# phlash/java-sdr

Hardware: AMD Instinct MI355X
Metric: IQ Msamples/s through FFT+FIR+BPSK demod, 2048-pt frames (higher is better)
Workload: dtype f64

## Files before the change

### java-sdr_amd/build.py

```python
#!/usr/bin/env python3
import os
import subprocess
import sys
from concurrent.futures import ThreadPoolExecutor

HERE = os.path.dirname(os.path.abspath(__file__))
CSRC = os.path.join(HERE, "csrc")
OBJ = os.path.join(HERE, "build")
OUT = os.path.join(HERE, "libjsdr_hip.so")

COMMON = ["--offload-arch=gfx950", "-O3", "-std=c++17", "-fPIC", "-Wall", "-Wno-unused-function",
          "-Wno-unused-result"]
SOURCES = {
    "bpsk_front_reg.hip": ["-ffp-contract=off"],
    "bpsk_fm.hip": ["-ffp-contract=off"],
    "bpsk_fm_f32.hip": ["-ffp-contract=off"],
    "bpsk_front.hip": ["-ffp-contract=off"],
    "bpsk_tail.hip": ["-ffp-contract=off"],
    "runtime.hip": [],
    "fft_psd.hip": [],
    "fft_mixed.hip": [],
    "fft_any.hip": ["-ffp-contract=off"],
    "fft_rt.hip": [],
    "fir_phase.hip": ["-ffp-contract=off"],
    "fir_batch.hip": ["-ffp-contract=off"],
    "fec.hip": [],
    "synth.hip": [],
    "formats.hip": [],
    "demod.hip": ["-ffp-contract=off"],
    "demod_chan.hip": ["-ffp-contract=off"],
    "bpsk_handle.hip": ["-ffp-contract=off"],
    "bpsk_sched.hip": ["-ffp-contract=off"],
    "bpsk_fft.hip": ["-ffp-contract=off"],
    "bpsk_acq.hip": ["-ffp-contract=off", "-mllvm", "-amdgpu-atomic-optimizer-strategy=None"],
    "bpsk_acq_chan.hip": ["-ffp-contract=off", "-mllvm", "-amdgpu-atomic-optimizer-strategy=None"],
    "bpsk_fftm.hip": ["-ffp-contract=off"],
    "bpsk_acqg.hip": ["-ffp-contract=off"],
    "bpsk_chan.hip": ["-ffp-contract=off"],
    "bpsk_pst.hip": ["-ffp-contract=off"],
# ... 57 lines not shown
```

### java-sdr_amd/csrc/bpsk_fm.hip

```cpp
#include "bpsk_units.h"
#include "bpsk_tuner.h"
#include <math.h>
#include <type_traits>
#include <stddef.h>
#include <stdlib.h>

namespace jsdr {
namespace fm { __constant__ BpskConst c_bpsk; }
using fm::c_bpsk;
}
#include "bpsk_matched.h"

namespace jsdr {


template <bool FAST>
__global__ __launch_bounds__(512) void k_matched(MatchedArgs a)
{
    extern __shared__ __align__(16) unsigned char smem[];
    double2 *X = reinterpret_cast<double2 *>(smem);
    const int s = blockIdx.y;
    const long long G = a.tile0 + 4160LL * blockIdx.x;
    const double2 *dm = a.dm + (long long)s * a.dm_stride;
    {
// ... 42 lines not shown
__global__ __launch_bounds__(64) void k_dm_history(double2 *dm, long long dm_stride, long long nds, int nstreams)
{
    int s = blockIdx.x;
    if (s >= nstreams) return;
    double2 *p = dm + (long long)s * dm_stride;
    double2 v = p[nds + threadIdx.x];
    __builtin_amdgcn_fence(__ATOMIC_RELEASE, "wavefront");
    __builtin_amdgcn_wave_barrier();
    asm volatile("s_waitcnt vmcnt(0)" ::: "memory");
    p[threadIdx.x] = v;
}


#ifdef JSDR_X_CLK
__device__ unsigned long long g_fm_clk[256][64];
#define FM_CLK(i)                                                                          \
    do {                                                                                   \
        const unsigned long long now_ = __builtin_amdgcn_s_memtime();                      \
        clk_acc_[i] += now_ - clk_last_;                                                   \
        clk_last_ = now_;                                                                  \
    } while (0)
#else
#define FM_CLK(i) do {} while (0)
#endif

__global__ void k_fm_edges(EdgeArgs a)
{
    const int t = blockIdx.x * blockDim.x + threadIdx.x;
    const int s = t / (4 * FM_EDGE), i = t % (4 * FM_EDGE);
    if (s >= a.nstreams) return;
    const int n = i < 2 * FM_EDGE ? i - FM_EDGE : a.nsamples - FM_EDGE + (i - 2 * FM_EDGE);
    int w = 0;
    if (n >= 0 && n < a.nsamples) {
        w = a.raw[(long long)s * a.stride_pairs + n];
    } else if (n < 0 && n >= -26) {
        w = a.hist[(long long)s * 32 + 26 + n].x;
        if (a.dc) {
            const int si = (int)(short)((w & 0xffff) - a.ic);
            const int sq = (int)(short)((w >> 16) - a.qc);
            w = (si & 0xffff) | (sq << 16);
        }
    }
    a.edges[(long long)s * (4 * FM_EDGE) + i] = w;
}

__global__ void k_fm_prep(EdgeArgs e, HistArgs hi, ScatterArgs sc)
// ... 48 lines not shown
        if (k != (float)(int)k || k >= 16384.0f || k <= -16384.0f) return false;
    }
    return true;
}
static_assert(ds_taps_are_short(), "dsFilter: every tap times 2^15 is an integer of magnitude below 2^14 (k_fm's +-1.0 fmas are exact)");

template <int D, int R, bool MIX, bool DC, bool FAST, bool SMALL = false, int PH = -1>
#ifndef JSDR_FM_MINWAVES
#define JSDR_FM_MINWAVES 2
#endif
__global__ __launch_bounds__(FM_THREADS, JSDR_FM_MINWAVES) void k_fm(FmArgs a)
{
    constexpr int RD = D * R, NS = RD - D + 27, NSQ = (NS + 3) / 4;
    constexpr int JOBS = (FM_NT + R - 1) / R, ROUNDS = (JOBS + FM_THREADS - 1) / FM_THREADS;
    static_assert(PH < 0 || (MIX && !FAST && PH < 4 && (D * R) % 8 == 0 && (65 * FM_NB * D) % 8 == 4),
                  "k_fm<PH>: the lane span is whole periods and a tile is half a period past the one before");
    extern __shared__ __align__(16) unsigned char smem[];
    double2 *X = reinterpret_cast<double2 *>(smem);
    double *sc = reinterpret_cast<double *>(smem + FM_NT * sizeof(double2));
    for (int i = threadIdx.x; i < 512; i += FM_THREADS) sc[i] = a.sincos[i];
#ifdef JSDR_X_CLK
    unsigned long long clk_acc_[6] = {0, 0, 0, 0, 0, 0}, clk_last_ = 0;
#endif
    const long long nwork = (long long)a.ntiles * a.nstreams;
#pragma unroll 1
    for (long long work = blockIdx.x; work < nwork; work += gridDim.x) {
    const int s = (int)(work / a.ntiles);
    const long long G = a.tile0 + (long long)(65 * FM_NB) * (work % a.ntiles);
    const int jrel0 = (int)(G - 64 - a.g_first);
#ifdef JSDR_X_FM_SMALLSET
    const int *raw = a.raw + (long long)(s & 15) * a.stride_pairs;
#else
    const int *raw = a.raw + (long long)s * a.stride_pairs;
#endif
    const int *edges = a.edges + (long long)s * (4 * FM_EDGE);
    const double2 *dmh_old = a.dmh_old + (long long)s * 64;
    const int Lm1 = a.nsamples - 1, nds = a.nds, P = a.tper;
    const double HOWARD = 0.9 * 32768.0 * (double)I16_2P15_UNSCALE;
    int e0 = 0;
    if constexpr (MIX) {
        const long long v = (long long)a.first_out + (long long)D * jrel0;
        e0 = (int)(((v % P) + P) % P);
    }
    typedef const __attribute__((address_space(4))) double *const_tab_t;
    const_tab_t tb = (const_tab_t)(a.tcs + e0);
    float amx = 0.0f;
    __syncthreads();
#ifdef JSDR_X_CLK
    clk_last_ = __builtin_amdgcn_s_memtime();
// ... 122 lines not shown
#pragma unroll 1
            for (int r = 0; r < R; r++) {
                const int t = t0 + r, j = j0 + r;
                const double2 val = (j >= -64 && j < 0) ? dmh_old[64 + j] : make_double2(0.0, 0.0);
                if (t < FM_NT) X[t] = val;
            }
        }
    }
    };
    if constexpr (PH < 0) {
        front(std::integral_constant<int, -1>{});
    } else {
        if (((e0 + a.trot) & 7) == PH) front(std::integral_constant<int, PH>{});
        else front(std::integral_constant<int, PH + 4>{});
    }
    if constexpr (FAST) {
#pragma unroll
        for (int off = 32; off >= 1; off >>= 1) amx = fmaxf(amx, __shfl_xor(amx, off, 64));
        if ((threadIdx.x & 63) == 0 && amx > 0.0f) atomicMax(a.amax + s, __float_as_int(amx));
    }
    FM_CLK(1);
    __syncthreads();
    FM_CLK(3);
    if (jrel0 + FM_NT > nds - 64) {
        double2 *dmh_new = a.dmh_new + (long long)s * 64;
        for (int t = 64 + threadIdx.x; t < FM_NT; t += FM_THREADS) {
            const int j = jrel0 + t;
            if (j >= nds - 64 && j < nds && j >= 0) dmh_new[j - (nds - 64)] = X[t];
        }
        if (work % a.ntiles == 0 && nds < 64 && (int)threadIdx.x < 64 - nds) dmh_new[threadIdx.x] = dmh_old[threadIdx.x + nds];
    }
    const int lane = threadIdx.x & 63;
    const int wave = __builtin_amdgcn_readfirstlane(threadIdx.x >> 6);
    const int blk = lane < FM_NB ? lane : FM_NB - 1;
    const double2 *xl = X + 64 + 65 * blk;
    const int rel0 = jrel0 + 64 + 65 * blk;
    double2 *y = a.y + (long long)s * a.y_stride;
    if constexpr (SMALL) {
        const int rel = (int)threadIdx.x, t = rel - jrel0;
        if (rel < nds && t >= 64 && t < FM_NT) {
            const long long g = a.g_first + rel;
            const int u = (int)(((g - 64) % 65 + 65) % 65);
            const double2 *xg = X + t;
            const double *f = c_bpsk.dm_taps;
            double yi = 0.0, yq = 0.0;
            for (int i = 0; i <= 64 - u; i++) {
// ... 56 lines not shown
    }
#else
    if (wave == 0) {
        double ai[9], aq[9];
        matched_block<9, FAST>(xl, 0, ai, aq);
#pragma unroll
        for (int r = 0; r < 9; r++) {
            const int rel = rel0 + r;
            if (lane < FM_NB && rel >= 0 && rel < nds) y[rel] = make_double2(ai[r], aq[r]);
        }
    } else {
        const int u0 = 9 + 8 * (wave - 1);
        double ai[8], aq[8];
        matched_block<8, FAST>(xl, u0, ai, aq);
#pragma unroll
        for (int r = 0; r < 8; r++) {
            const int rel = rel0 + u0 + r;
            if (lane < FM_NB && rel >= 0 && rel < nds) y[rel] = make_double2(ai[r], aq[r]);
        }
    }
#endif
    }
    FM_CLK(4);
    __syncthreads();
    FM_CLK(5);
    }
#ifdef JSDR_X_CLK
    if ((threadIdx.x & 63) == 0)
        for (int i = 0; i < 6; i++) atomicAdd(&g_fm_clk[blockIdx.x & 255][(threadIdx.x >> 6) * 8 + i], clk_acc_[i]);
#endif
}


int bpsk_fm_upload_constants(const BpskConst &bc)
{
    JSDR_HIP_TRY(hipMemcpyToSymbol(HIP_SYMBOL(c_bpsk), &bc, sizeof(bc)));
    return JSDR_OK;
}

int launch_matched(const MatchedArgs &ma, int nstreams, hipStream_t st)
{
    const long long ntiles = (ma.g_first + ma.nds - ma.tile0 + 4159) / 4160;
    const size_t lds = (64 + 4160) * sizeof(double2);
    JSDR_LDS_ATTR(k_matched<false>, lds);
    JSDR_LDS_ATTR(k_matched<true>, lds);
    hipLaunchKernelGGL(k_matched<false>, dim3((unsigned)ntiles, (unsigned)nstreams), dim3(512), lds, st, ma);
    return launched();
}

int launch_dm_history(double2 *dm, long long dm_stride, long long nds, int nstreams, hipStream_t st)
{
    hipLaunchKernelGGL(k_dm_history, dim3((unsigned)nstreams), dim3(64), 0, st, dm, dm_stride, nds, nstreams);
    return launched();
}

int launch_fm_prep(const EdgeArgs &ea, const HistArgs &ha, const ScatterArgs &sc, hipStream_t st)
{
    hipLaunchKernelGGL(k_fm_prep, dim3((unsigned)(((long long)ea.nstreams * (4 * FM_EDGE + 32) + sc.bytes[0] + sc.bytes[1] + 255) / 256)),
                       dim3(256), 0, st, ea, ha, sc);
    return launched();
}

template <int D, int R>
static int launch_fm_t(const FmArgs &a_in, bool mix, bool dc, bool fast, int nstreams, hipStream_t st, long long *items, long long *grid_out,
                       int *phase)
{
    *phase = -1;
    const size_t lds = (size_t)FM_NT * sizeof(double2) + 512 * sizeof(double);
    const long long span = 65LL * FM_NB;
    const long long ntiles = (a_in.g_first + a_in.nds - a_in.tile0 + span - 1) / span;
    FmArgs a = a_in;
    a.ntiles = (int)ntiles;
    a.nstreams = nstreams;
    static const long long grid_cap = [] {
        const char *e = knob("JSDR_FM_GRID");
        return e ? atoll(e) : 0LL;
    }();
    long long gx = ntiles * nstreams;
    if (grid_cap > 0 && gx > grid_cap) gx = grid_cap;
    if (a.grid_limit > 0 && gx > a.grid_limit) gx = a.grid_limit;
    *items = ntiles * nstreams;
    *grid_out = gx;
    const dim3 grid((unsigned)gx), block(FM_THREADS);
#define JSDR_FM_LAUNCH_PH(MIX, DC, FAST, SMALL, PH)                                                             \
    do {                                                                                                        \
        JSDR_LDS_ATTR((k_fm<D, R, MIX, DC, FAST, SMALL, PH>), lds);                                             \
        hipLaunchKernelGGL((k_fm<D, R, MIX, DC, FAST, SMALL, PH>), grid, block, lds, st, a);                    \
    } while (0)
#define JSDR_FM_LAUNCH(MIX, DC, FAST, SMALL) JSDR_FM_LAUNCH_PH(MIX, DC, FAST, SMALL, -1)
    const bool small = !fast && a.nds <= FM_THREADS && ntiles == 1;
    if constexpr (D == 10) {
        if (mix && !fast && !small && a.trot >= 0 && a.tper == 8) {
            const long long v = (long long)a.first_out + (long long)D * (a.tile0 - 64 - a.g_first);
            const int p0 = (int)((((v % 8) + 8) % 8 + a.trot) & 7);
            *phase = p0;
            switch (p0 & 3) {
                case 0: if (dc) JSDR_FM_LAUNCH_PH(true, true, false, false, 0); else JSDR_FM_LAUNCH_PH(true, false, false, false, 0); break;
                case 1: if (dc) JSDR_FM_LAUNCH_PH(true, true, false, false, 1); else JSDR_FM_LAUNCH_PH(true, false, false, false, 1); break;
                case 2: if (dc) JSDR_FM_LAUNCH_PH(true, true, false, false, 2); else JSDR_FM_LAUNCH_PH(true, false, false, false, 2); break;
                default: if (dc) JSDR_FM_LAUNCH_PH(true, true, false, false, 3); else JSDR_FM_LAUNCH_PH(true, false, false, false, 3); break;
            }
            return launched();
        }
    }
    if (small && a.nds <= FM_THREADS && ntiles == 1) {
// ... 6 lines not shown
        if (mix) { if (dc) JSDR_FM_LAUNCH(true, true, false, false); else JSDR_FM_LAUNCH(true, false, false, false); }
        else { if (dc) JSDR_FM_LAUNCH(false, true, false, false); else JSDR_FM_LAUNCH(false, false, false, false); }
    }
#undef JSDR_FM_LAUNCH
#undef JSDR_FM_LAUNCH_PH
    return launched();
}

int launch_fm(const FmArgs &a, int decim, bool mix, bool dc, bool fast, int nstreams, hipStream_t st, long long *items, long long *grid,
              int *phase)
{
    switch (decim) {
        case 4: return launch_fm_t<4, 5>(a, mix, dc, fast, nstreams, st, items, grid, phase);
        case 5: return launch_fm_t<5, 4>(a, mix, dc, fast, nstreams, st, items, grid, phase);
        case 10: return launch_fm_t<10, 4>(a, mix, dc, fast, nstreams, st, items, grid, phase);
        case 20: return launch_fm_t<20, 4>(a, mix, dc, fast, nstreams, st, items, grid, phase);
    }
    set_error("bpsk: unsupported decimation %d", decim);
    return JSDR_ERR;
}

void bpsk_fm_clocks_report()
{
#ifdef JSDR_X_CLK
    {
        static unsigned long long cc[256][64];
        if (hipMemcpyFromSymbol(cc, HIP_SYMBOL(g_fm_clk), sizeof(cc)) == hipSuccess) {
            static const char *nm[6] = {"-", "front half", "-", "barrier front", "matched", "barrier matched"};
            for (int i = 0; i < 6; i++) {
                if (i == 0 || i == 2) continue;
                fprintf(stderr, "k_fm clk %-16s", nm[i]);
                for (int w = 0; w < 8; w++) {
                    unsigned long long c = 0, tot = 0;
                    for (int b = 0; b < 256; b++) {
                        c += cc[b][w * 8 + i];
                        for (int k = 0; k < 6; k++) tot += cc[b][w * 8 + k];
                    }
                    fprintf(stderr, " w%d %5.1f%%", w, 100.0 * c / (tot ? tot : 1));
                }
                fprintf(stderr, "\n");
            }
            memset(cc, 0, sizeof(cc));
            hipMemcpyToSymbol(HIP_SYMBOL(g_fm_clk), cc, sizeof(cc));
        }
    }
#endif
// ... 4 lines not shown
```

### java-sdr_amd/csrc/bpsk_fm_f32.hip

```cpp
#include "bpsk_units.h"
#include <math.h>
#include <stddef.h>
#include <stdlib.h>

namespace jsdr {
namespace fm32 { __constant__ BpskConst c_bpsk; }
using fm32::c_bpsk;
}
#include "bpsk_matched.h"

namespace jsdr {

#ifndef JSDR_FM32_PQ
#define JSDR_FM32_PQ 6
#endif
enum { FM32_PQ = JSDR_FM32_PQ };

__global__ void k_fm_prep_f32(EdgeF32Args e, HistArgs hi)
{
    const int t = blockIdx.x * blockDim.x + threadIdx.x;
    const int nedge = e.nstreams * 4 * FM_EDGE;
    if (t < nedge) {
        const int s = t / (4 * FM_EDGE), i = t % (4 * FM_EDGE);
        const int n = i < 2 * FM_EDGE ? i - FM_EDGE : e.nsamples - FM_EDGE + (i - 2 * FM_EDGE);
// ... 14 lines not shown
    int2 v;
    if (n < 0) {
        v = hi.hist_old[(long long)s * 32 + (26 + n)];
    } else {
        const float2 f = hi.rawf[(long long)s * hi.stride_pairs + n];
        v = make_int2(__float_as_int(f.x), __float_as_int(f.y));
    }
    hi.hist_new[(long long)s * 32 + i] = v;
}

template <int D, int R, bool MIX, bool SMALL = false>
__global__ __launch_bounds__(FM_THREADS, 2) void k_fm_f32(FmF32Args fa)
{
    const FmArgs &a = fa.a;
    constexpr int RD = D * R, NS = RD - D + 27, NQ = (NS + 1) / 2;
    constexpr int PQ = FM32_PQ, NP = (NQ + PQ - 1) / PQ;
    constexpr int JOBS = (FM_NT + R - 1) / R, ROUNDS = (JOBS + FM_THREADS - 1) / FM_THREADS;
    static_assert(2 * NQ <= FM_EDGE, "a window must fit an edge image's half");
    extern __shared__ __align__(16) unsigned char smem[];
    double2 *X = reinterpret_cast<double2 *>(smem);
    double *sc = reinterpret_cast<double *>(smem + FM_NT * sizeof(double2));
    for (int i = threadIdx.x; i < 512; i += FM_THREADS) sc[i] = a.sincos[i];
    const long long nwork = (long long)a.ntiles * a.nstreams;
#pragma unroll 1
    for (long long work = blockIdx.x; work < nwork; work += gridDim.x) {
    const int s = (int)(work / a.ntiles);
    const long long G = a.tile0 + (long long)(65 * FM_NB) * (work % a.ntiles);
    const int jrel0 = (int)(G - 64 - a.g_first);
    const float2 *raw = fa.rawf + (long long)s * a.stride_pairs;
    const float2 *edges = fa.edges + (long long)s * (4 * FM_EDGE);
    const double2 *dmh_old = a.dmh_old + (long long)s * 64;
    const int Lm1 = a.nsamples - 1, nds = a.nds, P = a.tper;
    const double HOWARD = 0.9 * 32768.0;
    int e0 = 0;
    if constexpr (MIX) {
        const long long v = (long long)a.first_out + (long long)D * jrel0;
        e0 = (int)(((v % P) + P) % P);
    }
    typedef const __attribute__((address_space(4))) double *const_tab_t;
    const_tab_t tb = (const_tab_t)(a.tcs + e0);
    __syncthreads();
#pragma unroll 1
    for (int round = 0; round < ROUNDS; round++) {
        const int job = threadIdx.x + FM_THREADS * round;
        const int t0 = R * job;
        if (t0 >= FM_NT) break;
        const int j0 = jrel0 + t0;
        const int n0 = a.first_out + D * j0 - 26;
// ... 100 lines not shown
#pragma unroll 1
                for (int r = 0; r < R; r++) {
                    const int t = t0 + r, j = j0 + r;
                    double2 val = make_double2(0.0, 0.0);
                    if (j >= 0 && j < nds) {
                        val.x = r == 0 ? oi[0] : r == 1 ? oi[1] : r == 2 ? oi[2] : r == 3 ? oi[3] : oi[R - 1];
                        val.y = r == 0 ? oq[0] : r == 1 ? oq[1] : r == 2 ? oq[2] : r == 3 ? oq[3] : oq[R - 1];
                    } else if (j >= -64 && j < 0) {
                        val = dmh_old[64 + j];
                    }
                    if (t < FM_NT) X[t] = val;
                }
            }
        } else {
#pragma unroll 1
            for (int r = 0; r < R; r++) {
                const int t = t0 + r, j = j0 + r;
                const double2 val = (j >= -64 && j < 0) ? dmh_old[64 + j] : make_double2(0.0, 0.0);
                if (t < FM_NT) X[t] = val;
            }
        }
    }
    __syncthreads();
    if (jrel0 + FM_NT > nds - 64) {
        double2 *dmh_new = a.dmh_new + (long long)s * 64;
        for (int t = 64 + threadIdx.x; t < FM_NT; t += FM_THREADS) {
            const int j = jrel0 + t;
            if (j >= nds - 64 && j < nds && j >= 0) dmh_new[j - (nds - 64)] = X[t];
        }
        if (work % a.ntiles == 0 && nds < 64 && (int)threadIdx.x < 64 - nds) dmh_new[threadIdx.x] = dmh_old[threadIdx.x + nds];
    }
    const int lane = threadIdx.x & 63;
    const int wave = __builtin_amdgcn_readfirstlane(threadIdx.x >> 6);
    const int blk = lane < FM_NB ? lane : FM_NB - 1;
    const double2 *xl = X + 64 + 65 * blk;
    double2 *y = a.y + (long long)s * a.y_stride;
    if constexpr (SMALL) {
        const int rel = (int)threadIdx.x, t = rel - jrel0;
        if (rel < nds && t >= 64 && t < FM_NT) {
            const long long g = a.g_first + rel;
            const int u = (int)(((g - 64) % 65 + 65) % 65);
            const double2 *xg = X + t;
            const double *f = c_bpsk.dm_taps;
            double yi = 0.0, yq = 0.0;
            for (int i = 0; i <= 64 - u; i++) {
                const double2 x = xg[-(u + i)];
// ... 18 lines not shown
            u0 = 9 + 8 * (wave - 1);
            nout = 8;
            double bi[8], bq[8];
            matched_block<8, false>(xl, u0, bi, bq);
#pragma unroll
            for (int r = 0; r < 8; r++) {
                ai[r] = bi[r];
                aq[r] = bq[r];
            }
        }
        __syncthreads();
        if (lane < FM_NB) {
#pragma unroll
            for (int r = 0; r < 9; r++)
                if (r < nout) X[65 * blk + u0 + r] = make_double2(ai[r], aq[r]);
        }
        __syncthreads();
        const int relb = jrel0 + 64;
        for (int o = (int)threadIdx.x; o < 65 * FM_NB; o += FM_THREADS) {
            const int rel = relb + o;
            if (rel >= 0 && rel < nds) y[rel] = X[o];
        }
    }
    __syncthreads();
    }
}

int bpsk_fm_f32_upload_constants(const BpskConst &bc)
{
    JSDR_HIP_TRY(hipMemcpyToSymbol(HIP_SYMBOL(c_bpsk), &bc, sizeof(bc)));
    return JSDR_OK;
}

int launch_fm_prep_f32(const EdgeF32Args &ea, const HistArgs &ha, hipStream_t st)
{
    hipLaunchKernelGGL(k_fm_prep_f32, dim3((unsigned)(((long long)ea.nstreams * (4 * FM_EDGE + 32) + 255) / 256)), dim3(256), 0, st, ea, ha);
    return launched();
}

template <int D, int R>
static int launch_fm_f32_t(const FmF32Args &a_in, bool mix, int nstreams, hipStream_t st, long long *items, long long *grid_out)
{
    const size_t lds = (size_t)FM_NT * sizeof(double2) + 512 * sizeof(double);
    const long long span = 65LL * FM_NB;
    const long long ntiles = (a_in.a.g_first + a_in.a.nds - a_in.a.tile0 + span - 1) / span;
    FmF32Args a = a_in;
    a.a.ntiles = (int)ntiles;
    a.a.nstreams = nstreams;
    long long gx = ntiles * nstreams;
    if (a.a.grid_limit > 0 && gx > a.a.grid_limit) gx = a.a.grid_limit;
    *items = ntiles * nstreams;
    *grid_out = gx;
    const dim3 grid((unsigned)gx), block(FM_THREADS);
#define JSDR_FM32_LAUNCH(MIX, SMALL)                                              \
    do {                                                                          \
        JSDR_LDS_ATTR((k_fm_f32<D, R, MIX, SMALL>), lds);                         \
        hipLaunchKernelGGL((k_fm_f32<D, R, MIX, SMALL>), grid, block, lds, st, a); \
    } while (0)
    if (a.a.nds <= FM_THREADS && ntiles == 1) {
        if (mix) JSDR_FM32_LAUNCH(true, true); else JSDR_FM32_LAUNCH(false, true);
    } else {
        if (mix) JSDR_FM32_LAUNCH(true, false); else JSDR_FM32_LAUNCH(false, false);
    }
#undef JSDR_FM32_LAUNCH
    return launched();
}

int launch_fm_f32(const FmF32Args &a, int decim, bool mix, int nstreams, hipStream_t st, long long *items, long long *grid)
{
    switch (decim) {
        case 4: return launch_fm_f32_t<4, 5>(a, mix, nstreams, st, items, grid);
        case 5: return launch_fm_f32_t<5, 4>(a, mix, nstreams, st, items, grid);
        case 10: return launch_fm_f32_t<10, 4>(a, mix, nstreams, st, items, grid);
        case 20: return launch_fm_f32_t<20, 4>(a, mix, nstreams, st, items, grid);
    }
// ... 6 lines not shown
```

### java-sdr_amd/csrc/bpsk_handle.hip

```cpp
#include "bpsk_kernels.h"
#include "bpsk_fec.h"
#include "bpsk_fft.h"
#include "bpsk_chan.h"
#include "bpsk_pst.h"
#include "bpsk_sched.h"
#include "bpsk_blob.h"
#include "bpsk_state.h"
#include <math.h>
#include <cmath>
#include <atomic>
#include <memory>
#include <thread>
#include <stddef.h>
#include <stdlib.h>
#include <vector>

static const float h_ds_half[14] = {-6.103515625000e-004F, -1.220703125000e-004F, +2.380371093750e-003F,
                                    +6.164550781250e-003F, +7.324218750000e-003F, +7.629394531250e-004F,
                                    -1.464843750000e-002F, -3.112792968750e-002F, -3.225708007813e-002F,
                                    -1.617431640625e-003F, +6.463623046875e-002F, +1.502380371094e-001F,
                                    +2.231445312500e-001F, +2.518310546875e-001F};
static const float h_dm_half[33] = {
    -0.0101130691F, -0.0086975143F, -0.0038246093F, +0.0033563764F, +0.0107237026F, +0.0157790936F, +0.0164594107F,
    +0.0119213911F, +0.0030315224F, -0.0076488191F, -0.0164594107F, -0.0197184277F, -0.0150109226F, -0.0023082460F,
// ... 36 lines not shown
    Schedule cur, prefetch;
    bool tables_on_device = false;
    unsigned char h_khist[26] = {0};
    bool retuned = false;
    bool fft_ready = false;
    int seam = 0;
    DevBuf<FftFrontState> fft_state2;
    DevBuf<double2> dm2;
    long long dm2_stride = 0;
    unsigned char h_mhist[26] = {0};
    DevBuf<unsigned short> ktu9;
    DevBuf<double> sincos9;
    std::vector<unsigned short> h_ktu9;
    int c_kshift = -1;
    DevBuf<double> sincos;
    DevBuf<unsigned char> ktu;
    DevBuf<unsigned char> kvco;
    DevBuf<int2> hist_in[2];
    int hist_cur = 0;
    bool hist_is_float = false;
    DevBuf<int> hist_bad;
    DevBuf<int> amax;
    DevBuf<SnapPack> snap_dev;
    DevBuf<int> fm_edges;
    DevBuf<float2> fm_edges_f32;
    bool f32_batch = false;
    DevBuf<double2> dm, y[2];
    int y_cur = 0;
    DevBuf<double2> dmh[2], tcs;
    int dmh_cur = 0;
    int tab_cur = 0;
    bool halo_in_dmh = false;
    bool use_fm = true;
    long long last_fm_items = 0, last_fm_grid = 0;
    int last_fm_phase = -1;
    int share_wgs_per_cu = 0;
    int num_cu = 0;
    int variant = 0;
    double fast_ey = 0.0;
    double margin_scale = 1.0;
    double argmax_scale = 1.0;
    const char *front_name = "k_front";
    const char *tail_name = "k_tail";
    const char *fec_name = "k_fec_bpsk";
    bool ktu_uploaded = false;
    std::thread worker;
// ... 1193 lines not shown
    } else if (nds > 0 && fm_ok) {
        if (wait_tail(h, h->y_cur, st) != JSDR_OK) return JSDR_ERR;
        FmArgs ma;
        ma.raw = fa.raw;
        ma.stride_pairs = fa.stride_pairs;
        ma.nsamples = (int)L;
        ma.ic = ic;
        ma.qc = qc;
        ma.edges = h->fm_edges.p;
        ma.tcs = tcs_p;
        ma.tper = h->cur.mix ? h->cur.tper : 1;
        ma.kvco = kvco_p;
        ma.sincos = h->sincos.p;
        ma.dmh_old = h->dmh[h->dmh_cur].p;
        ma.dmh_new = h->dmh[h->dmh_cur ^ 1].p;
        ma.y = h->y[h->y_cur].p + Y_PAD;
        ma.y_stride = h->y_stride;
        ma.nds = (int)nds;
        ma.g_first = g_first;
        ma.tile0 = first_block(g_first);
        ma.first_out = first_out;
        ma.amax = h->amax.p;
        ma.grid_limit = h->share_wgs_per_cu * h->num_cu;
        ma.trot = h->cur.mix == 1 ? h->cur.trot : -1;
        if (rawf_dev) {
            EdgeF32Args ea;
            ea.rawf = fa.rawf;
            ea.stride_pairs = fa.stride_pairs;
            ea.nsamples = (int)L;
            ea.hist = fa.hist;
            ea.edges = h->fm_edges_f32.p;
            ea.nstreams = S;
            const HistArgs ha = hist_args(h, nullptr, fa.rawf, fa.stride_pairs, L, 0, 0, S);
            ProfScope psh(h, PK_PREP, st);
            if (launch_fm_prep_f32(ea, ha, st) != JSDR_OK) return JSDR_ERR;
            hist_done = true;
        } else {
            EdgeArgs ea;
            ea.raw = fa.raw;
            ea.stride_pairs = fa.stride_pairs;
            ea.nsamples = (int)L;
            ea.ic = ic;
            ea.qc = qc;
            ea.dc = (ic != 0) || (qc != 0);
            ea.hist = fa.hist;
            ea.edges = h->fm_edges.p;
// ... 212 lines not shown
    if (const char *e = knob("JSDR_NO_OVERLAP")) h->overlap = atoi(e) == 0;
    if (const char *e = knob("JSDR_FM")) h->use_fm = atoi(e) != 0;
    if (const char *e = knob("JSDR_SCHED_PREFETCH")) h->prefetch_on = atoi(e) != 0;
    const size_t S = (size_t)nstreams;
    bool vitq = nstreams >= 256;
    if (const char *e = knob("JSDR_VITQ")) vitq = atoi(e) != 0 && nstreams > 1;
    h->dm_stride = 64 + h->max_ds + 64;
    h->y_stride = h->max_ds;
    h->bitlog_stride = (HIST_BITS + h->max_bits + 64 + 15) & ~15LL;
    bool ok = h->sincos.alloc(512) == JSDR_OK && h->ktu.alloc((size_t)h->max_batch + 8192) == JSDR_OK &&
              h->kvco.alloc(2 * (size_t)h->max_ds) == JSDR_OK && h->hist_in[0].alloc(S * 32) == JSDR_OK &&
              h->hist_in[1].alloc(S * 32) == JSDR_OK && h->dm.alloc(S * (size_t)h->dm_stride) == JSDR_OK &&
              h->y[0].alloc(S * (size_t)h->y_stride + 2 * Y_PAD) == JSDR_OK && h->y[1].alloc(S * (size_t)h->y_stride + 2 * Y_PAD) == JSDR_OK && h->tail.alloc(S) == JSDR_OK &&
              h->bitlog[0].alloc(S * (size_t)h->bitlog_stride) == JSDR_OK &&
              h->bitlog[1].alloc(S * (size_t)h->bitlog_stride) == JSDR_OK && h->nbits.alloc(S) == JSDR_OK &&
              h->trig_count.alloc(S) == JSDR_OK && h->trig_bits.alloc(S * h->trig_cap) == JSDR_OK &&
              h->fec_scratch.alloc(vitq ? (size_t)fec_vitq_scratch_words(nstreams, h->trig_cap) : S * h->trig_cap * (size_t)fec_dec_scratch_words()) == JSDR_OK && h->fec_done.alloc(S) == JSDR_OK &&
              (!vitq || (h->fec_vit.alloc(S * h->trig_cap * 320) == JSDR_OK && h->fec_work.alloc(S * h->trig_cap + 1) == JSDR_OK)) &&
              h->fec_rc.alloc(S * h->trig_cap) == JSDR_OK && h->fec_last.alloc(S * 2) == JSDR_OK &&
              h->cnt_dec.alloc(S) == JSDR_OK && h->corr.alloc(S * (size_t)h->max_bits) == JSDR_OK &&
              h->fec_data.alloc(S * h->trig_cap * 256) == JSDR_OK && h->decoded.alloc(S * 256) == JSDR_OK &&
              h->stage_raw.alloc((size_t)nsamples_per_frame * 2 + (nstreams == 1 ? ((do_fft ? sizeof(double2) : 1) * (size_t)h->max_ds + sizeof(double2) * (256 + FM_TABLE_SLACK) + 256) / 4 : 0)) == JSDR_OK &&
              h->ds_taps_dev.alloc(32) == JSDR_OK &&
              h->dmh[0].alloc(S * 64) == JSDR_OK && h->dmh[1].alloc(S * 64) == JSDR_OK && h->hist_bad.alloc(1) == JSDR_OK && h->amax.alloc(S) == JSDR_OK && h->fm_edges.alloc(S * 4 * FM_EDGE) == JSDR_OK && h->snap_dev.alloc(1) == JSDR_OK && h->tcs.alloc(2 * (256 + FM_TABLE_SLACK)) == JSDR_OK;
    if (ok && nstreams == 1) {
        const size_t need = sizeof(float) * 2 * (size_t)nsamples_per_frame + ((size_t)h->max_batch + 26) + (size_t)h->max_ds +
                            (do_fft ? sizeof(double2) * (size_t)h->max_ds : 0) + sizeof(double2) * (256 + FM_TABLE_SLACK) + 8 * 64;
        const size_t arena = (need + 63) & ~(size_t)63;
        if (arena <= ((size_t)8 << 20) && h->pin.alloc(arena + sizeof(SnapPack))) h->pin_bytes = arena;
        else (void)hipGetLastError();
    }
    if (!ok) {
        jsdr_bpsk_destroy(h);
        return JSDR_ERR;
    }
    std::vector<double> sc(512);
    for (int n = 0; n < 256; n++) {
        sc[n] = table_cos(n);
        sc[256 + n] = table_sin(n);
    }
    BpskConst bc;
    memset(&bc, 0, sizeof(bc));
    double sync[SYNC_N];
    (void)jsdr_bpsk_table(0, bc.ds_taps, 32);
    (void)jsdr_bpsk_table(1, bc.dm_taps, 96);
    (void)jsdr_bpsk_table(2, sync, SYNC_N);
    for (int i = 0; i < SYNC_N; i++) bc.sync[i] = sync[i] > 0.0 ? 1 : -1;
// ... 1534 lines not shown
```

### java-sdr_amd/csrc/bpsk_kernels.h

```cpp
#pragma once
#include "common.h"
#include "bpsk_fft.h"

namespace jsdr {

enum { DS_N = 27, DM_N = 65, HIST_BITS = 5200, MIN_TRIG = 8, SYNC_N = 65 };
enum { Y_PAD = 1024 };
#ifndef JSDR_FM_NB
#define JSDR_FM_NB 62
#endif
enum { FM_NB = JSDR_FM_NB, FM_NT = 64 + 65 * FM_NB, FM_THREADS = 512, FM_TABLE_SLACK = 128, FM_EDGE = 128 };

struct BpskConst {
    double ds_taps[32];
    double dm_taps[96];
    signed char sync[72];
};
int bpsk_upload_constants(const BpskConst &bc);

struct TailState {
    double dmEnergy[8];
    double dmEnergyOut;
    double lastI, lastQ;
    double energy1, energy2;
// ... 58 lines not shown
};

struct FmArgs {
    const int *raw;
    long long stride_pairs;
    int nsamples;
    int ic, qc;
    const int *edges;
    const double2 *tcs;
    int tper;
    const unsigned char *kvco;
    const double *sincos;
    const double2 *dmh_old;
    double2 *dmh_new;
    double2 *y;
    long long y_stride;
    int nds;
    long long g_first;
    long long tile0;
    int first_out;
    int *amax;
    int ntiles, nstreams;
    int grid_limit;
    int trot;
};

struct EdgeArgs {
    const int *raw;
    long long stride_pairs;
    int nsamples, ic, qc, dc;
    const int2 *hist;
    int *edges;
    int nstreams;
};
struct ScatterArgs {
    const unsigned char *src[2];
    unsigned char *dst[2];
    int bytes[2];
};

struct FmF32Args {
    FmArgs a;
    const float2 *rawf;
    const float2 *edges;
};
struct EdgeF32Args {
// ... 91 lines not shown
```

### java-sdr_amd/csrc/fft_common.h

```cpp
#pragma once
#include "common.h"
#include <utility>
#include <vector>

namespace jsdr {

constexpr double cx_pi = 3.14159265358979323846264338327950288;

constexpr double cx_sin_small(double x)
{
    double x2 = x * x, term = x, sum = x;
    for (int i = 1; i < 12; i++) {
        term *= -x2 / ((2 * i) * (2 * i + 1));
        sum += term;
    }
    return sum;
}
constexpr double cx_cos_small(double x)
{
    double x2 = x * x, term = 1.0, sum = 1.0;
    for (int i = 1; i < 12; i++) {
        term *= -x2 / ((2 * i - 1) * (2 * i));
        sum += term;
    }
// ... 78 lines not shown
    int o = 0;
    for (int b = 1; b < r; b <<= 1) {
        o = (o << 1) | (v & 1);
        v >>= 1;
    }
    return o;
}

__device__ __forceinline__ int lds_pad(int idx) { return idx + (idx >> 4); }
constexpr int lds_frame_elems(int n) { return n + (n >> 4) + 1; }


enum { IN_I16 = 0, IN_F32 = 1 };
enum { OUT_PSD = 0, OUT_SPEC = 1 };

struct FftArgs {
    const void *in;
    float *out;
    const float2 *tw;
    long long nframes;
    int rate;
    int ic, qc;
    int split = 0;
};

struct Best {
    float v;
    int k;
};

struct MixedPlan {
    int n = 0, nrad = 0, radix[6] = {1, 1, 1, 1, 1, 1};
    int threads = 0;
    size_t lds_bytes = 0;
    int tw_count = 0;
    bool split2 = false;
    int half_tw_count = 0;
};
bool mixed_plan(int n, MixedPlan &p);
void mixed_twiddles(const MixedPlan &p, float2 *out);
int mixed_launch(const MixedPlan &p, const FftArgs &a, int in_kind, int out_kind, int grid, hipStream_t st);
int mixed_launch_split2(const MixedPlan &p, const FftArgs &a, int in_kind, int out_kind, int num_cu, hipStream_t st);

bool rt_supported(int n);
void rt_twiddles(int n, std::vector<float2> &w);
int rt_launch(const FftArgs &a, int n, int in_kind, int out_kind, int num_cu, hipStream_t st);
// ... 6 lines not shown
```

### java-sdr_amd/csrc/fft_psd.hip

```cpp
#include "fft_common.h"
#include <math.h>
#include <stdlib.h>
#include <vector>

namespace jsdr {

constexpr bool tw_direct(int P, int R) { return P * R <= 512; }
constexpr int tw_size(int P, int R) { return P <= 1 ? 0 : (tw_direct(P, R) ? 2 * P * (R - 1) : P); }
constexpr int tw_total(int R0, int R1, int R2, int R3)
{
    return tw_size(R0, R1) + (R2 > 1 ? tw_size(R0 * R1, R2) : 0) + (R3 > 1 ? tw_size(R0 * R1 * R2, R3) : 0);
}

constexpr int ilog2_c(int n) { return n <= 1 ? 0 : 1 + ilog2_c(n / 2); }

template <int R, int P>
__device__ __forceinline__ void apply_twiddles(float2 *v, int k, const float2 *tab)
{
    if constexpr (P > 1) {
        if constexpr (tw_direct(P, R)) {
#pragma unroll
            for (int r = 1; r < R; r++) {
                const float4 t = reinterpret_cast<const float4 *>(tab)[(r - 1) * P + k];
                v[r] = cmul2(v[r], make_float2(t.x, t.y), make_float2(t.z, t.w));
// ... 193 lines not shown
                for (int w = 1; w < NW; w++) {
                    float ov = red_val[frame_in_block * NW + w];
                    int ok = red_idx[frame_in_block * NW + w];
                    if (ov > bestv || (ov == bestv && ok < bestk)) {
                        bestv = ov;
                        bestk = ok;
                    }
                }
            }
        }
        if (tid == 0 && active) {
            int p = (bestv > -3.402823466e+38f) ? 2 * bestk : -1;
            float m = (p >= 0) ? bestv : -3.402823466e+38f;
            const int datlen = 2 * N;
            if (p >= datlen / 2) p -= datlen;
            int hz = (int)((unsigned)p * (unsigned)a.rate) / datlen;
            float *dst = a.out + frame * (N + 2);
            dst[N] = (float)hz;
            dst[N + 1] = m;
        }
    }
}

template <int N, int T, int FPB, int IN, int OUT, int R0, int R1, int R2, int R3, bool TWG = false>
__global__ __launch_bounds__(T *FPB, (N == 2048 ? 4 : 1)) void k_fft(FftArgs a)
{
    extern __shared__ __align__(16) unsigned char smem[];
    constexpr int FE = lds_frame_elems(N);
    constexpr int TWN = TWG ? 0 : tw_total(R0, R1, R2, R3);
    float2 *tw_own = reinterpret_cast<float2 *>(smem);
    float2 *bufs = tw_own + TWN;
    float *red_val = reinterpret_cast<float *>(bufs + (size_t)FPB * FE);
    int *red_idx = reinterpret_cast<int *>(red_val + FPB * ((T + 63) / 64));
    const float2 *tw_lds = TWG ? a.tw : tw_own;

    const int tid_b = threadIdx.x;
    if constexpr (!TWG) {
        for (int i = tid_b; i < TWN; i += T * FPB) tw_own[i] = a.tw[i];
        __syncthreads();
    }

    const int fib = tid_b / T;
    const int tid = tid_b - fib * T;
    float2 *buf = bufs + (size_t)fib * FE;
    const long long ngroups = (a.nframes + FPB - 1) / FPB;
    auto frame_of = [&](long long g) {
        long long f = g * FPB + fib;
        return f < a.nframes ? f : a.nframes - 1;
    };
    typename RawPoint<IN>::type raw[R0];
    if ((long long)blockIdx.x < ngroups) fft_fetch<N, T, IN, R0>(a, frame_of(blockIdx.x), tid, raw);
    for (long long g = blockIdx.x; g < ngroups; g += gridDim.x) {
        const long long gn = g + gridDim.x;
        fft_frame<N, T, IN, OUT, R0, R1, R2, R3>(a, frame_of(g), frame_of(gn < ngroups ? gn : g), tid, buf, tw_lds, red_val,
                                                 red_idx, fib, raw);
        __syncthreads();
    }
}

template <int N, int FPB, int T, int R0, int R1, int R2, int R3, bool TWG = false>
constexpr size_t fft_lds_bytes()
{
    return sizeof(float2) * ((TWG ? (size_t)0 : (size_t)tw_total(R0, R1, R2, R3)) + (size_t)FPB * lds_frame_elems(N)) +
           (sizeof(float) + sizeof(int)) * FPB * ((T + 63) / 64);
}

struct Launcher {
    void (*launch)(const FftArgs &, int grid, hipStream_t) = nullptr;
    int frames_per_block = 0;
    size_t lds_bytes = 0;
    int block = 0;
    int radix[4] = {1, 1, 1, 1};
};

template <int N, int T, int FPB, int IN, int OUT, int R0, int R1, int R2, int R3, bool TWG = false>
static void launch_impl(const FftArgs &a, int grid, hipStream_t s)
{
    constexpr size_t lds = fft_lds_bytes<N, FPB, T, R0, R1, R2, R3, TWG>();
    hipLaunchKernelGGL((k_fft<N, T, FPB, IN, OUT, R0, R1, R2, R3, TWG>), dim3(grid), dim3(T * FPB), lds, s, a);
}
// ... 31 lines not shown
}

}

using namespace jsdr;

struct jsdr_fft {
    int n = 0;
    int rate = 0;
    DevBuf<float2> tw;
    DevBuf<float2> tw_i16;
    DevBuf<unsigned char> in_stage;
    DevBuf<float> out_stage;
    PinnedStage pin;
    bool pin_lazy_done = false;
    int num_cu = 256;
    bool mixed = false;
    MixedPlan mplan;
    bool rt = false;
    bool direct = false;
    long long last_items = 0, last_grid = 0;
    int share_wgs_per_cu = 0;
};

static int fft_run(jsdr_fft *h, const void *in_dev, int in_kind, int out_kind, long long nframes, int ic, int qc,
                   float *out_dev, hipStream_t s)
{
    JSDR_REQUIRE(h, "fft: null handle");
    JSDR_REQUIRE(in_dev && out_dev, "fft: null buffer");
    JSDR_REQUIRE(nframes >= 0, "fft: negative frame count");
    if (nframes == 0) return JSDR_OK;
    FftArgs a;
    if (h->rt) {
        a.in = in_dev;
        a.out = out_dev;
        a.tw = h->tw.p;
        a.nframes = nframes;
        a.rate = h->rate;
        a.ic = ic;
        a.qc = qc;
        return rt_launch(a, h->n, in_kind, out_kind, h->num_cu, s);
    }
    if (h->direct) {
        a.in = in_dev;
        a.out = out_dev;
        a.tw = nullptr;
// ... 25 lines not shown
    a.nframes = nframes;
    a.rate = h->rate;
    a.ic = ic;
    a.qc = qc;
    long long groups = (nframes + l.frames_per_block - 1) / l.frames_per_block;
    long long per_cu = (long long)(160 * 1024 / l.lds_bytes);
    if (per_cu < 1) per_cu = 1;
    if (per_cu * l.block > 2048) per_cu = 2048 / l.block;
    static const int mult = [] {
        const char *e = knob("JSDR_FFT_GRID_MULT");
        const int v = e ? atoi(e) : 0;
        return v > 0 ? v : 4;
    }();
    long long cap = (long long)h->num_cu * per_cu * mult;
    static const int abs_grid = [] {
        const char *e = knob("JSDR_FFT_GRID_ABS");
        return e ? atoi(e) : 0;
    }();
    if (abs_grid > 0) cap = abs_grid;
    if (h->share_wgs_per_cu > 0) cap = (long long)h->num_cu * h->share_wgs_per_cu;
    int grid = (int)(groups < cap ? groups : cap);
    h->last_items = groups;
    h->last_grid = grid;
    l.launch(a, grid, s);
    JSDR_LAUNCH_CHECK();
    return JSDR_OK;
}

extern "C" {

int jsdr_fft_create(jsdr_fft **out, int n, int rate)
{
    JSDR_REQUIRE(out, "jsdr_fft_create: null handle pointer");
    *out = nullptr;
    MixedPlan mp;
    const bool pow2 = n >= 64 && n <= 8192 && (n & (n - 1)) == 0;
    const bool mixed = !pow2 && mixed_plan(n, mp);
    const bool rt = !pow2 && !mixed && rt_supported(n);
    const bool direct = !pow2 && !mixed && !rt && dft_any_supported(n);
    JSDR_REQUIRE(pow2 || mixed || rt || direct,
                 "jsdr_fft_create: n=%d unsupported (2 .. 20000 samples)", n);
    JSDR_REQUIRE(rate > 0, "jsdr_fft_create: rate must be positive");
    int dev = 0;
    JSDR_HIP_TRY(hipGetDevice(&dev));
    hipDeviceProp_t prop;
    JSDR_HIP_TRY(hipGetDeviceProperties(&prop, dev));
// ... 67 lines not shown
        return JSDR_ERR;
    }
    std::vector<float2> tw16(tw);
    if (fft_i16_scaled(l.radix[0], l.radix[1]))
        for (int i = 0; i < tw_size(l.radix[0], l.radix[1]); i++)
            tw16[i] = make_float2(tw16[i].x * I16_2P15_UNSCALE, tw16[i].y * I16_2P15_UNSCALE);
    if (h->tw.alloc(tw.size()) != JSDR_OK || h->tw_i16.alloc(tw16.size()) != JSDR_OK ||
        h->in_stage.alloc((size_t)n * 8) != JSDR_OK || h->out_stage.alloc((size_t)n + 2) != JSDR_OK) {
        jsdr_fft_destroy(h);
        return JSDR_ERR;
    }
    if (hipMemcpy(h->tw.p, tw.data(), sizeof(float2) * tw.size(), hipMemcpyHostToDevice) != hipSuccess ||
        hipMemcpy(h->tw_i16.p, tw16.data(), sizeof(float2) * tw16.size(), hipMemcpyHostToDevice) != hipSuccess) {
        set_error("jsdr_fft_create: twiddle upload failed");
        jsdr_fft_destroy(h);
        return JSDR_ERR;
    }
    *out = h;
    return JSDR_OK;
}

int jsdr_fft_destroy(jsdr_fft *h)
{
    delete h;
    return JSDR_OK;
}

int jsdr_fft_batch_f32(jsdr_fft *h, const float *iq_dev, int64_t nframes, float *psd_dev, void *stream)
{
    return fft_run(h, iq_dev, IN_F32, OUT_PSD, nframes, 0, 0, psd_dev, as_stream(stream));
}

int jsdr_fft_set_cu_share(jsdr_fft *h, int wgs_per_cu)
{
    JSDR_REQUIRE(h && wgs_per_cu >= 0 && wgs_per_cu <= 16, "jsdr_fft_set_cu_share: bad argument");
    h->share_wgs_per_cu = wgs_per_cu;
    return JSDR_OK;
}

const char *jsdr_fft_kernel(jsdr_fft *h)
{
    if (!h) return "";
    return h->rt ? "k_fft_rt" : h->direct ? "k_dft_any" : h->mixed ? (h->mplan.split2 ? "k_fft_mixed_dual" : "k_fft_mixed") : "k_fft";
}

int jsdr_fft_last_launch(jsdr_fft *h, int64_t *work_items, int64_t *workgroups)
// ... 60 lines not shown
```

Baseline: 241,600.

## Use atomic ticket work-stealing for persistent FM kernel tiles when grid is capped

Replaces the static grid-stride tile assignment in the persistent FM kernels (f64 and f32) with dynamic tickets from a global atomic counter, broadcast through an LDS slot. This applies only when a CU-share grid limit caps the grid below the work count. The aim is to balance uneven per-tile work across workgroups and cut tail idle time, at the cost of one atomic per tile and a memset per launch. It also adds compile-gated per-workgroup clock instrumentation for FM and FFT.

```diff
diff --git a/java-sdr_amd/build.py b/java-sdr_amd/build.py
--- a/java-sdr_amd/build.py
+++ b/java-sdr_amd/build.py
@@ -13,8 +13,8 @@
           "-Wno-unused-result"]
 SOURCES = {
     "bpsk_front_reg.hip": ["-ffp-contract=off"],
-    "bpsk_fm.hip": ["-ffp-contract=off"],
-    "bpsk_fm_f32.hip": ["-ffp-contract=off"],
+    "bpsk_fm.hip": ["-ffp-contract=off", "-mllvm", "-amdgpu-atomic-optimizer-strategy=None"],
+    "bpsk_fm_f32.hip": ["-ffp-contract=off", "-mllvm", "-amdgpu-atomic-optimizer-strategy=None"],
     "bpsk_front.hip": ["-ffp-contract=off"],
     "bpsk_tail.hip": ["-ffp-contract=off"],
     "runtime.hip": [],
diff --git a/java-sdr_amd/csrc/bpsk_fm.hip b/java-sdr_amd/csrc/bpsk_fm.hip
--- a/java-sdr_amd/csrc/bpsk_fm.hip
+++ b/java-sdr_amd/csrc/bpsk_fm.hip
@@ -88,6 +88,12 @@
     } while (0)
 #else
 #define FM_CLK(i) do {} while (0)
+#endif
+
+#ifdef JSDR_X_WGCLK
+constexpr int WGCLK_SLOTS = 128, WGCLK_WGS = 1024;
+__device__ unsigned long long g_fm_wgclk[WGCLK_SLOTS][WGCLK_WGS][3];
+static long long g_wgclk_log[WGCLK_SLOTS][4];
 #endif
 
 __global__ void k_fm_edges(EdgeArgs a)
@@ -182,9 +188,15 @@
 #ifdef JSDR_X_CLK
     unsigned long long clk_acc_[6] = {0, 0, 0, 0, 0, 0}, clk_last_ = 0;
 #endif
+#ifdef JSDR_X_WGCLK
+    const unsigned long long wgclk0 = __builtin_amdgcn_s_memrealtime();
+    unsigned long long wgclk_n = 0;
+#endif
     const long long nwork = (long long)a.ntiles * a.nstreams;
+    const bool tickets = a.tickets != nullptr;
+    int *tkL = reinterpret_cast<int *>(sc + 512);
 #pragma unroll 1
-    for (long long work = blockIdx.x; work < nwork; work += gridDim.x) {
+    for (long long work = blockIdx.x; work < nwork; work = tickets ? (long long)gridDim.x + (unsigned)__builtin_amdgcn_readfirstlane(tkL[0]) : work + gridDim.x) {
     const int s = (int)(work / a.ntiles);
     const long long G = a.tile0 + (long long)(65 * FM_NB) * (work % a.ntiles);
     const int jrel0 = (int)(G - 64 - a.g_first);
@@ -353,6 +365,8 @@
     FM_CLK(1);
     __syncthreads();
     FM_CLK(3);
+    unsigned tk = 0;
+    if (tickets && threadIdx.x == 0) tk = atomicAdd(a.tickets, 1u);
     if (jrel0 + FM_NT > nds - 64) {
         double2 *dmh_new = a.dmh_new + (long long)s * 64;
         for (int t = 64 + threadIdx.x; t < FM_NT; t += FM_THREADS) {
@@ -455,9 +469,25 @@
 #endif
     }
     FM_CLK(4);
+    {
+        int zlate = 0;
+        asm volatile("" : "+v"(zlate));
+        if (tickets && threadIdx.x == 0) tkL[0] = (int)tk + zlate;
+    }
     __syncthreads();
     FM_CLK(5);
-    }
+#ifdef JSDR_X_WGCLK
+    wgclk_n++;
+#endif
+    }
+#ifdef JSDR_X_WGCLK
+    if (threadIdx.x == 0 && blockIdx.x < WGCLK_WGS) {
+        unsigned long long *c = g_fm_wgclk[a.wgclk_slot][blockIdx.x];
+        c[0] = wgclk0;
+        c[1] = __builtin_amdgcn_s_memrealtime();
+        c[2] = wgclk_n;
+    }
+#endif
 #ifdef JSDR_X_CLK
     if ((threadIdx.x & 63) == 0)
         for (int i = 0; i < 6; i++) atomicAdd(&g_fm_clk[blockIdx.x & 255][(threadIdx.x >> 6) * 8 + i], clk_acc_[i]);
@@ -499,7 +529,7 @@
                        int *phase)
 {
     *phase = -1;
-    const size_t lds = (size_t)FM_NT * sizeof(double2) + 512 * sizeof(double);
+    const size_t lds = (size_t)FM_NT * sizeof(double2) + 512 * sizeof(double) + sizeof(double);
     const long long span = 65LL * FM_NB;
     const long long ntiles = (a_in.g_first + a_in.nds - a_in.tile0 + span - 1) / span;
     FmArgs a = a_in;
@@ -514,6 +544,20 @@
     if (a.grid_limit > 0 && gx > a.grid_limit) gx = a.grid_limit;
     *items = ntiles * nstreams;
     *grid_out = gx;
+    if (!(a.grid_limit > 0 && gx < ntiles * nstreams && ntiles * nstreams + gx < 0x7fffffffLL)) a.tickets = nullptr;
+#ifdef JSDR_X_WGCLK
+    {
+        static int wgclk_seq = 0;
+        static const bool wgclk_static = getenv("JSDR_X_WGCLK_STATIC") != nullptr;
+        if (wgclk_static) a.tickets = nullptr;
+        a.wgclk_slot = wgclk_seq % WGCLK_SLOTS;
+        g_wgclk_log[a.wgclk_slot][0] = ntiles * nstreams;
+        g_wgclk_log[a.wgclk_slot][1] = gx;
+        g_wgclk_log[a.wgclk_slot][2] = a.tickets != nullptr;
+        g_wgclk_log[a.wgclk_slot][3] = wgclk_seq++;
+    }
+#endif
+    if (a.tickets) JSDR_HIP_TRY(hipMemsetAsync(a.tickets, 0, sizeof(unsigned), st));
     const dim3 grid((unsigned)gx), block(FM_THREADS);
 #define JSDR_FM_LAUNCH_PH(MIX, DC, FAST, SMALL, PH)                                                             \
     do {                                                                                                        \
@@ -566,6 +610,21 @@
 
 void bpsk_fm_clocks_report()
 {
+#ifdef JSDR_X_WGCLK
+    {
+        const char *path = getenv("JSDR_X_WGCLK_OUT_FM");
+        FILE *f = fopen(path ? path : "wgclk_fm.csv", "w");
+        static unsigned long long cc[WGCLK_SLOTS][WGCLK_WGS][3];
+        if (f && hipMemcpyFromSymbol(cc, HIP_SYMBOL(g_fm_wgclk), sizeof(cc)) == hipSuccess) {
+            fprintf(f, "launch,items,grid,ticket,wg,t0,t1,n\n");
+            for (int sl = 0; sl < WGCLK_SLOTS; sl++)
+                for (int w = 0; w < WGCLK_WGS && w < g_wgclk_log[sl][1]; w++)
+                    fprintf(f, "%lld,%lld,%lld,%lld,%d,%llu,%llu,%llu\n", g_wgclk_log[sl][3], g_wgclk_log[sl][0], g_wgclk_log[sl][1],
+                            g_wgclk_log[sl][2], w, cc[sl][w][0], cc[sl][w][1], cc[sl][w][2]);
+        }
+        if (f) fclose(f);
+    }
+#endif
 #ifdef JSDR_X_CLK
     {
         static unsigned long long cc[256][64];
diff --git a/java-sdr_amd/csrc/bpsk_fm_f32.hip b/java-sdr_amd/csrc/bpsk_fm_f32.hip
--- a/java-sdr_amd/csrc/bpsk_fm_f32.hip
+++ b/java-sdr_amd/csrc/bpsk_fm_f32.hip
@@ -60,8 +60,10 @@
     double *sc = reinterpret_cast<double *>(smem + FM_NT * sizeof(double2));
     for (int i = threadIdx.x; i < 512; i += FM_THREADS) sc[i] = a.sincos[i];
     const long long nwork = (long long)a.ntiles * a.nstreams;
+    const bool tickets = a.tickets != nullptr;
+    int *tkL = reinterpret_cast<int *>(sc + 512);
 #pragma unroll 1
-    for (long long work = blockIdx.x; work < nwork; work += gridDim.x) {
+    for (long long work = blockIdx.x; work < nwork; work = tickets ? (long long)gridDim.x + (unsigned)__builtin_amdgcn_readfirstlane(tkL[0]) : work + gridDim.x) {
     const int s = (int)(work / a.ntiles);
     const long long G = a.tile0 + (long long)(65 * FM_NB) * (work % a.ntiles);
     const int jrel0 = (int)(G - 64 - a.g_first);
@@ -208,6 +210,8 @@
         }
     }
     __syncthreads();
+    unsigned tk = 0;
+    if (tickets && threadIdx.x == 0) tk = atomicAdd(a.tickets, 1u);
     if (jrel0 + FM_NT > nds - 64) {
         double2 *dmh_new = a.dmh_new + (long long)s * 64;
         for (int t = 64 + threadIdx.x; t < FM_NT; t += FM_THREADS) {
@@ -272,6 +276,11 @@
             if (rel >= 0 && rel < nds) y[rel] = X[o];
         }
     }
+    {
+        int zlate = 0;
+        asm volatile("" : "+v"(zlate));
+        if (tickets && threadIdx.x == 0) tkL[0] = (int)tk + zlate;
+    }
     __syncthreads();
     }
 }
@@ -291,7 +300,7 @@
 template <int D, int R>
 static int launch_fm_f32_t(const FmF32Args &a_in, bool mix, int nstreams, hipStream_t st, long long *items, long long *grid_out)
 {
-    const size_t lds = (size_t)FM_NT * sizeof(double2) + 512 * sizeof(double);
+    const size_t lds = (size_t)FM_NT * sizeof(double2) + 512 * sizeof(double) + sizeof(double);
     const long long span = 65LL * FM_NB;
     const long long ntiles = (a_in.a.g_first + a_in.a.nds - a_in.a.tile0 + span - 1) / span;
     FmF32Args a = a_in;
@@ -301,6 +310,8 @@
     if (a.a.grid_limit > 0 && gx > a.a.grid_limit) gx = a.a.grid_limit;
     *items = ntiles * nstreams;
     *grid_out = gx;
+    if (!(a.a.grid_limit > 0 && gx < ntiles * nstreams && ntiles * nstreams + gx < 0x7fffffffLL)) a.a.tickets = nullptr;
+    if (a.a.tickets) JSDR_HIP_TRY(hipMemsetAsync(a.a.tickets, 0, sizeof(unsigned), st));
     const dim3 grid((unsigned)gx), block(FM_THREADS);
 #define JSDR_FM32_LAUNCH(MIX, SMALL)                                              \
     do {                                                                          \
diff --git a/java-sdr_amd/csrc/bpsk_handle.hip b/java-sdr_amd/csrc/bpsk_handle.hip
--- a/java-sdr_amd/csrc/bpsk_handle.hip
+++ b/java-sdr_amd/csrc/bpsk_handle.hip
@@ -82,6 +82,7 @@
     DevBuf<int> hist_bad;
     DevBuf<int> amax;
     DevBuf<SnapPack> snap_dev;
+    DevBuf<unsigned> fm_tickets;
     DevBuf<int> fm_edges;
     DevBuf<float2> fm_edges_f32;
     bool f32_batch = false;
@@ -1321,6 +1322,7 @@
         ma.first_out = first_out;
         ma.amax = h->amax.p;
         ma.grid_limit = h->share_wgs_per_cu * h->num_cu;
+        ma.tickets = h->fm_tickets.p;
         ma.trot = h->cur.mix == 1 ? h->cur.trot : -1;
         if (rawf_dev) {
             EdgeF32Args ea;
@@ -1579,7 +1581,7 @@
               h->fec_data.alloc(S * h->trig_cap * 256) == JSDR_OK && h->decoded.alloc(S * 256) == JSDR_OK &&
               h->stage_raw.alloc((size_t)nsamples_per_frame * 2 + (nstreams == 1 ? ((do_fft ? sizeof(double2) : 1) * (size_t)h->max_ds + sizeof(double2) * (256 + FM_TABLE_SLACK) + 256) / 4 : 0)) == JSDR_OK &&
               h->ds_taps_dev.alloc(32) == JSDR_OK &&
-              h->dmh[0].alloc(S * 64) == JSDR_OK && h->dmh[1].alloc(S * 64) == JSDR_OK && h->hist_bad.alloc(1) == JSDR_OK && h->amax.alloc(S) == JSDR_OK && h->fm_edges.alloc(S * 4 * FM_EDGE) == JSDR_OK && h->snap_dev.alloc(1) == JSDR_OK && h->tcs.alloc(2 * (256 + FM_TABLE_SLACK)) == JSDR_OK;
+              h->dmh[0].alloc(S * 64) == JSDR_OK && h->dmh[1].alloc(S * 64) == JSDR_OK && h->hist_bad.alloc(1) == JSDR_OK && h->amax.alloc(S) == JSDR_OK && h->fm_tickets.alloc(1) == JSDR_OK && h->fm_edges.alloc(S * 4 * FM_EDGE) == JSDR_OK && h->snap_dev.alloc(1) == JSDR_OK && h->tcs.alloc(2 * (256 + FM_TABLE_SLACK)) == JSDR_OK;
     if (ok && nstreams == 1) {
         const size_t need = sizeof(float) * 2 * (size_t)nsamples_per_frame + ((size_t)h->max_batch + 26) + (size_t)h->max_ds +
                             (do_fft ? sizeof(double2) * (size_t)h->max_ds : 0) + sizeof(double2) * (256 + FM_TABLE_SLACK) + 8 * 64;
diff --git a/java-sdr_amd/csrc/bpsk_kernels.h b/java-sdr_amd/csrc/bpsk_kernels.h
--- a/java-sdr_amd/csrc/bpsk_kernels.h
+++ b/java-sdr_amd/csrc/bpsk_kernels.h
@@ -104,6 +104,10 @@
     int *amax;
     int ntiles, nstreams;
     int grid_limit;
+    unsigned *tickets;
+#ifdef JSDR_X_WGCLK
+    int wgclk_slot;
+#endif
     int trot;
 };
 
diff --git a/java-sdr_amd/csrc/fft_common.h b/java-sdr_amd/csrc/fft_common.h
--- a/java-sdr_amd/csrc/fft_common.h
+++ b/java-sdr_amd/csrc/fft_common.h
@@ -124,6 +124,9 @@
     int rate;
     int ic, qc;
     int split = 0;
+#ifdef JSDR_X_WGCLK
+    int wgclk_slot = 0;
+#endif
 };
 
 struct Best {
diff --git a/java-sdr_amd/csrc/fft_psd.hip b/java-sdr_amd/csrc/fft_psd.hip
--- a/java-sdr_amd/csrc/fft_psd.hip
+++ b/java-sdr_amd/csrc/fft_psd.hip
@@ -239,6 +239,11 @@
     }
 }
 
+#ifdef JSDR_X_WGCLK
+constexpr int WGCLK_SLOTS = 128, WGCLK_WGS = 1024;
+__device__ unsigned long long g_fft_wgclk[WGCLK_SLOTS][WGCLK_WGS][3];
+#endif
+
 template <int N, int T, int FPB, int IN, int OUT, int R0, int R1, int R2, int R3, bool TWG = false>
 __global__ __launch_bounds__(T *FPB, (N == 2048 ? 4 : 1)) void k_fft(FftArgs a)
 {
@@ -250,6 +255,10 @@
     float *red_val = reinterpret_cast<float *>(bufs + (size_t)FPB * FE);
     int *red_idx = reinterpret_cast<int *>(red_val + FPB * ((T + 63) / 64));
     const float2 *tw_lds = TWG ? a.tw : tw_own;
+#ifdef JSDR_X_WGCLK
+    const unsigned long long wgclk0 = __builtin_amdgcn_s_memrealtime();
+    unsigned long long wgclk_n = 0;
+#endif
 
     const int tid_b = threadIdx.x;
     if constexpr (!TWG) {
@@ -272,7 +281,18 @@
         fft_frame<N, T, IN, OUT, R0, R1, R2, R3>(a, frame_of(g), frame_of(gn < ngroups ? gn : g), tid, buf, tw_lds, red_val,
                                                  red_idx, fib, raw);
         __syncthreads();
-    }
+#ifdef JSDR_X_WGCLK
+        wgclk_n++;
+#endif
+    }
+#ifdef JSDR_X_WGCLK
+    if (tid_b == 0 && blockIdx.x < WGCLK_WGS) {
+        unsigned long long *c = g_fft_wgclk[a.wgclk_slot][blockIdx.x];
+        c[0] = wgclk0;
+        c[1] = __builtin_amdgcn_s_memrealtime();
+        c[2] = wgclk_n;
+    }
+#endif
 }
 
 template <int N, int FPB, int T, int R0, int R1, int R2, int R3, bool TWG = false>
@@ -350,6 +370,24 @@
     long long last_items = 0, last_grid = 0;
     int share_wgs_per_cu = 0;
 };
+
+#ifdef JSDR_X_WGCLK
+static long long g_wgclk_log[WGCLK_SLOTS][3];
+static void fft_wgclk_report()
+{
+    const char *path = getenv("JSDR_X_WGCLK_OUT");
+    FILE *f = fopen(path ? path : "wgclk_fft.csv", "w");
+    static unsigned long long cc[WGCLK_SLOTS][WGCLK_WGS][3];
+    if (f && hipMemcpyFromSymbol(cc, HIP_SYMBOL(g_fft_wgclk), sizeof(cc)) == hipSuccess) {
+        fprintf(f, "launch,items,grid,ticket,wg,t0,t1,n\n");
+        for (int sl = 0; sl < WGCLK_SLOTS; sl++)
+            for (int w = 0; w < WGCLK_WGS && w < g_wgclk_log[sl][1]; w++)
+                fprintf(f, "%lld,%lld,%lld,0,%d,%llu,%llu,%llu\n", g_wgclk_log[sl][2], g_wgclk_log[sl][0], g_wgclk_log[sl][1], w,
+                        cc[sl][w][0], cc[sl][w][1], cc[sl][w][2]);
+    }
+    if (f) fclose(f);
+}
+#endif
 
 static int fft_run(jsdr_fft *h, const void *in_dev, int in_kind, int out_kind, long long nframes, int ic, int qc,
                    float *out_dev, hipStream_t s)
@@ -421,6 +459,15 @@
     int grid = (int)(groups < cap ? groups : cap);
     h->last_items = groups;
     h->last_grid = grid;
+#ifdef JSDR_X_WGCLK
+    {
+        static int wgclk_seq = 0;
+        a.wgclk_slot = wgclk_seq % WGCLK_SLOTS;
+        g_wgclk_log[a.wgclk_slot][0] = groups;
+        g_wgclk_log[a.wgclk_slot][1] = grid;
+        g_wgclk_log[a.wgclk_slot][2] = wgclk_seq++;
+    }
+#endif
     l.launch(a, grid, s);
     JSDR_LAUNCH_CHECK();
     return JSDR_OK;
@@ -534,6 +581,12 @@
 
 int jsdr_fft_destroy(jsdr_fft *h)
 {
+#ifdef JSDR_X_WGCLK
+    if (h) {
+        (void)hipDeviceSynchronize();
+        fft_wgclk_report();
+    }
+#endif
     delete h;
     return JSDR_OK;
 }
```

After: 249,100 (median of 6 runs). +3.1%, better.
